# culiver/VAR

Hardware: AMD Instinct MI355X
Metric: 256x256 images/sec (CFG=1.5) VAR-d16 (higher is better)
Workload: dtype f32

## Files before the change

include/var_hip.h:

```cpp
#ifndef VAR_HIP_H
#define VAR_HIP_H

#include <stdint.h>

#ifdef __cplusplus
extern "C" {
#endif

#define VARHIP_EINVAL (-1)

typedef void* varhip_stream_t;

const char* varhip_version(void);

#define VARHIP_EPI_NONE 0
#define VARHIP_EPI_GELU 1
#define VARHIP_EPI_RESID 2
int varhip_gemm_nt_f32(const float* A, int64_t lda, const float* W, int64_t ldw, const float* bias,
                       float* out, int64_t ldo, int M, int N, int K, int epi,
                       const float* resid, int64_t ldr, const float* gamma, int64_t ldg, int rows_per_group,
                       int bias_per_row, int batch, int64_t sA, int64_t sW, int64_t sO, varhip_stream_t stream);

int varhip_silu_f32(const float* x, float* y, int64_t n, varhip_stream_t stream);

// ... 49 lines not shown
int varhip_upconv_pack_f32(const float* w, float* w_phase, int Cin, int Cout, varhip_stream_t stream);
int varhip_upconv_phase_f32(const float* in, const float* w_phase, const float* bias, float* out,
                            int B, int H, int W, int Cin, int Cout, varhip_stream_t stream);
int varhip_upconv_phase_gn_f32(const float* in, const float* w_phase, const float* bias, float* out, double* gn_part,
                               int B, int H, int W, int Cin, int Cout, varhip_stream_t stream);

int64_t varhip_gn_scratch_elems(int B, int HW, int C, int G);
int varhip_gn_stats_f32(const float* x, float* stats, double* scratch, int B, int HW, int C, int G, float eps, varhip_stream_t stream);
int varhip_gn_apply_f32(const float* x, const float* stats, const float* gamma, const float* beta, float* out,
                        int B, int HW, int C, int G, int silu, varhip_stream_t stream);

int varhip_gn_silu_conv_out_f32(const float* x, const float* stats, const float* gamma, const float* beta, const float* w, const float* bias,
                                float* out, int B, int H, int W, int Cin, int Cout, int G, int out_mode, varhip_stream_t stream);

int varhip_softmax_rows_f32(const float* x, float* out, int64_t rows, int n, float scale, varhip_stream_t stream);

int varhip_nchw_to_nhwc_f32(const float* in, float* out, int B, int C, int HW, varhip_stream_t stream);
int varhip_nhwc_to_nchw_f32(const float* in, float* out, int B, int C, int HW, varhip_stream_t stream);

int varhip_conv_gn_blocks(int H, int W, int Cout, int phase);
int varhip_conv3x3_gn_nhwc_f32(const float* in, const float* w, const float* bias, const float* resid, float* out, double* gn_part,
                               int B, int H, int W, int Cin, int Cout, int up2, varhip_stream_t stream);
int varhip_gn_stats_part_f32(const double* gn_part, float* stats, int B, int nblk, int HW, int C, int G, float eps, varhip_stream_t stream);
int varhip_conv3x3_s2_nhwc_f32(const float* in, const float* w, const float* bias, float* out,
                               int B, int H, int W, int Cin, int Cout, varhip_stream_t stream);
int varhip_nchw_to_nhwc_pad_f32(const float* in, float* out, int B, int C, int HW, int Cpad, varhip_stream_t stream);
int varhip_area_pool_f32(const float* f, float* pooled, int B, int P, int pq, int Cv, varhip_stream_t stream);
int varhip_word_embed_f32(const float* pooled, const float* word_w, const float* word_b, const float* lvl_pos,
                          float* x_out, int B, int lq, int C, int Cv, varhip_stream_t stream);
int varhip_quant_residual_f32(const int64_t* idx, const float* codebook, const int32_t* tap_idx, const float* tap_w,
                              const float* phi_w, const float* phi_b, float ratio, float* up, float* f_hat, float* f_rest,
                              int B, int pn, int P, int Cv, varhip_stream_t stream);

int varhip_token_select_i64(const uint8_t* keep, const int64_t* gt, const int64_t* sampled, int64_t* out, int64_t n, varhip_stream_t stream);

int varhip_neighbor_table_f32(const float* codebook, int V, int D, int n, int32_t* nbr_idx, float* nbr_dist, varhip_stream_t stream);
int varhip_smooth_select_f32(const float* logits, const int64_t* gt, const int32_t* nbr_idx, const float* nbr_dist, int n,
                             int cand_count, int use_thr, float thr, float ratio, int B, int l, int V, double t_cfg,
                             int64_t* idx_out, float* maxval_out, float* distlp_out, float* cfg_out, varhip_stream_t stream);

int varhip_token_loglik_f32(const float* logits, const int64_t* gt, int64_t ld_gt, int images, int classes, int l, int V,
                            int with_uncond, float ca, float cb, float* out, int64_t ld_out_img, int64_t ld_out_cls, varhip_stream_t stream);

int varhip_code_dist_f32(const float* codebook, int V, int D, float* out, varhip_stream_t stream);
int varhip_token_score_f32(const float* logits, const int64_t* gt, int64_t ld_gt, int images, int classes, int l, int V,
                           int with_uncond, float ca, float cb, int mode, int param, float thr, const float* dist, int64_t ld_dist,
// ... 56 lines not shown
                              void* out, int M, int C, int rows_per_group, float eps, varhip_stream_t stream);
int varhip_adaln_block_bf16(float* x, float* x2, void* xn16, void* q16, void* att16, void* hid16, const float* ada, int64_t ld_ada,
                           const void* qkv_w16, const float* qkv_b, const float* scale_mul, float plain_scale, int l2norm,
                           const void* proj_w16, const float* proj_b, const void* fc1_w16, const float* fc1_b,
                           const void* fc2_w16, const float* fc2_b, void* kcache16, void* vcache16,
                           int B2, int l, int C, int H, int hidden, int pos0, int Lmax, float eps, varhip_stream_t stream);
int varhip_conv3x3_nhwc_bf16(const void* in, const void* w, const float* bias, const void* resid, void* out, double* gn_part,
                            int B, int H, int W, int Cin, int Cout, int out_mode, varhip_stream_t stream);
int varhip_upconv_phase_bf16(const void* in, const void* w_phase, const float* bias, void* out, double* gn_part,
                            int B, int H, int W, int Cin, int Cout, varhip_stream_t stream);
int varhip_gnconv3x3_nhwc_bf16(const void* in, const float* table, int silu,
                               const void* w, const float* bias, const void* resid, void* out, double* gn_part,
                               int B, int H, int W, int Cin, int Cout, varhip_stream_t stream);
int varhip_conv16_force_tile(int wm);
int varhip_gn_stats_bf16(const void* x, float* stats, double* scratch, int B, int HW, int C, int G, float eps, varhip_stream_t stream);
int varhip_gn_apply_bf16(const void* x, const float* stats, const float* gamma, const float* beta, void* out,
                        int B, int HW, int C, int G, int silu, varhip_stream_t stream);
int varhip_gn_silu_conv_out_bf16(const void* x, const float* stats, const float* gamma, const float* beta, const void* w, const float* bias,
                                 float* out, int B, int H, int W, int Cin, int Cout, int G, int out_mode, varhip_stream_t stream);
int varhip_cast_f32_to_bf16(const float* in, void* out, int64_t n, varhip_stream_t stream);
int varhip_cast_bf16_to_f32(const void* in, float* out, int64_t n, varhip_stream_t stream);


#define VARHIP_NFAM 15
int varhip_timing_enable(int on);
int varhip_timing_select(int family_mask);
int varhip_timing_reset(void);
int varhip_timing_read(double* ms, double* flops, double* bytes, int64_t* launches);
const char* varhip_timing_name(int family);

#ifdef __cplusplus
}
#endif
#endif
```

var_amd/abi.py:

```python
import ctypes as C

P = C.c_void_p
I = C.c_int
L = C.c_int64
F = C.c_float
D = C.c_double

SIGNATURES = {
    'gemm_nt_f32':       [P, L, P, L, P, P, L, I, I, I, I, P, L, P, L, I, I, I, L, L, L],
    'silu_f32':          [P, P, L],
    'add_bcast_f32':     [P, P, P, I, I],
    'ln_modulate_f32':   [P, P, L, P, L, P, I, I, I, F],
    'qkv_prep_f32':      [P, P, F, I, P, P, P, I, I, I, I, I],
    'attn_cached_f32':   [P, P, P, P, I, I, I, I, I],
    'cfg_sample_f32':    [P, P, P, P, I, I, I, D, I, D],
    'quant_accum_f32':   [P, P, P, P, P, P, F, P, P, I, I, I, I],
    'next_map_f32':      [P, P, P, P, P, P, I, I, I, I, I],
    'lvl_pos_f32':       [P, P, P, P, I, I],
    'first_map_f32':     [P, P, I, P, P, P, P, I, I, I],
    'conv3x3_nhwc_f32':  [P, P, P, P, P, I, I, I, I, I, I, I],
    'gn_stats_f32':      [P, P, P, I, I, I, I, F],
    'gn_apply_f32':      [P, P, P, P, P, I, I, I, I, I],
    'softmax_rows_f32':  [P, P, L, I, F],
    'nchw_to_nhwc_f32':  [P, P, I, I, I],
# ... 21 lines not shown

SIGNATURES_F16 = {
    'gemm_nt_f16':       [P, L, P, L, P, P, L, I, I, I, I, I, P, L, I, P, L, I, I, L, L, L],
    'gemm_qkv_f16':      [P, L, P, L, P, I, I, I, P, F, I, P, P, P, I, I, I, I, I],
    'attn_cached_f16':   [P, P, P, P, I, I, I, I, I],
    'ln_modulate_f16out': [P, P, L, P, L, P, I, I, I, F],
    'adaln_block_f16':   [P, P, P, P, P, P, P, L, P, P, P, F, I, P, P, P, P, P, P, P, P, I, I, I, I, I, I, I, F],
    'conv3x3_nhwc_f16':  [P, P, P, P, P, P, I, I, I, I, I, I],
    'upconv_phase_f16':  [P, P, P, P, P, I, I, I, I, I],
    'gnconv3x3_nhwc_f16': [P, P, I, P, P, P, P, P, I, I, I, I, I],
    'gn_stats_f16':      [P, P, P, I, I, I, I, F],
    'gn_apply_f16':      [P, P, P, P, P, I, I, I, I, I],
    'gn_silu_conv_out_f16': [P, P, P, P, P, P, P, I, I, I, I, I, I, I],
    'cast_f32_to_f16':   [P, P, L],
    'cast_f16_to_f32':   [P, P, L],
}

SIGNATURES_HIP_ONLY = {
    'gn_scale_shift_f32': [P, P, P, P, I, I, I],
    'gn_silu_conv_out_f32': [P, P, P, P, P, P, P, I, I, I, I, I, I, I],
    'token_loglik_f32':  [P, P, L, I, I, I, I, I, F, F, P, L, L],
    'code_dist_f32':     [P, I, I, P],
    'token_score_f32':   [P, P, L, I, I, I, I, I, F, F, I, I, F, P, L, P, L, L],
}

SIGNATURES_BF16 = {k.replace('_f16out', '_bf16out').replace('_to_f16', '_to_bf16').replace('cast_f16_', 'cast_bf16_').replace('_f16', '_bf16'): v
                   for k, v in SIGNATURES_F16.items()}

EPI_NONE, EPI_GELU, EPI_RESID = 0, 1, 2
EINVAL = -1


def bind(lib, prefix: str, with_stream: bool):
    fns = {}
    table = dict(SIGNATURES)
    if with_stream:
        table.update(SIGNATURES_F16)
        table.update(SIGNATURES_BF16)
        table.update(SIGNATURES_HIP_ONLY)
    for name, args in table.items():
        fn = getattr(lib, prefix + name)
        fn.argtypes = list(args) + ([P] if with_stream else [])
        fn.restype = I
        fns[name] = fn
    gs = getattr(lib, prefix + 'gn_scratch_elems')
    gs.argtypes = [I, I, I, I]
# ... 17 lines not shown
```

var_amd/csrc/common.h:

```cpp
#pragma once
#include <hip/hip_runtime.h>
#include <stdint.h>
#include <stdlib.h>
#include "../../include/var_hip.h"
#include "../../include/var_math.h"

typedef float f32x2 __attribute__((ext_vector_type(2)));
__device__ __forceinline__ f32x2 vh_exp_pair(f32x2 x) {
    const f32x2 xc = {__builtin_fminf(x[0], 88.0f), __builtin_fminf(x[1], 88.0f)};
    const f32x2 t = xc * 1.44269504088896341f;
    const f32x2 n = {__builtin_rintf(t[0]), __builtin_rintf(t[1])};
    f32x2 r = __builtin_elementwise_fma(n, (f32x2)(-0.693145751953125f), xc);
    r = __builtin_elementwise_fma(n, (f32x2)(-1.42860682030941723212e-6f), r);
    f32x2 q = (f32x2)(1.9875691500e-4f);
    q = __builtin_elementwise_fma(q, r, (f32x2)(1.3981999507e-3f));
    q = __builtin_elementwise_fma(q, r, (f32x2)(8.3334519073e-3f));
    q = __builtin_elementwise_fma(q, r, (f32x2)(4.1665795894e-2f));
    q = __builtin_elementwise_fma(q, r, (f32x2)(1.6666665459e-1f));
    q = __builtin_elementwise_fma(q, r, (f32x2)(5.0000001201e-1f));
    const f32x2 y = __builtin_elementwise_fma(q, r * r, r) + 1.0f;
    f32x2 o;
    o[0] = (x[0] > -87.0f) ? __builtin_ldexpf(y[0], (int)n[0]) : 0.0f;
    o[1] = (x[1] > -87.0f) ? __builtin_ldexpf(y[1], (int)n[1]) : 0.0f;
    return o;
// ... 4 lines not shown
    const f32x2 u = (x + x3 * 0.044715f) * 0.7978845608028654f;
    const f32x2 d = vh_exp_pair(u * -2.0f) + 1.0f;
    return f32x2{x[0] / d[0], x[1] / d[1]};
}

typedef float f32x4 __attribute__((ext_vector_type(4)));
typedef float f32x16 __attribute__((ext_vector_type(16)));

#define VH_FAM_GEMM 0
#define VH_FAM_CONV 1
#define VH_FAM_ATTN 2
#define VH_FAM_SAMPLER 3
#define VH_FAM_LN 4
#define VH_FAM_QKV 5
#define VH_FAM_GN 6
#define VH_FAM_OTHER 7
#define VH_FAM_GEMM_SMALL 8
#define VH_FAM_CONV_SMALL 9
#define VH_FAM_GEMM16 10
#define VH_FAM_GEMM16_SMALL 11
#define VH_FAM_CONV16H 12
#define VH_FAM_CONV16_SMALL 13
#define VH_FAM_ATTN16 14

int vh_timing_on(int fam);
void vh_timing_begin(int fam, hipStream_t s, double flops, double bytes);
void vh_timing_end(int fam, hipStream_t s);

struct VhScope {
    int fam; hipStream_t s; bool on;
    VhScope(int f, hipStream_t st, double flops, double bytes) : fam(f), s(st), on(vh_timing_on(f) != 0) { if (on) vh_timing_begin(fam, s, flops, bytes); }
    ~VhScope() { if (on) vh_timing_end(fam, s); }
};

static inline int vh_launch_status() {
    hipError_t e = hipGetLastError();
    return e == hipSuccess ? 0 : -(1000 + (int)e);
}

template <int CTRL> __device__ __forceinline__ float vh_mov_dpp(float v) {
    return __int_as_float(__builtin_amdgcn_mov_dpp(__float_as_int(v), CTRL, 0xF, 0xF, true));
}
__device__ __forceinline__ float vh_lane_xor4(float v) {
    const float up = vh_mov_dpp<0x104>(v), dn = vh_mov_dpp<0x114>(v);
    return (threadIdx.x & 4) ? dn : up;
}
__device__ __forceinline__ float vh_wave_sum(float p) {
    { const auto r = __builtin_amdgcn_permlane32_swap(__float_as_uint(p), __float_as_uint(p), false, false); p = __uint_as_float(r[0]) + __uint_as_float(r[1]); }
    { const auto r = __builtin_amdgcn_permlane16_swap(__float_as_uint(p), __float_as_uint(p), false, false); p = __uint_as_float(r[0]) + __uint_as_float(r[1]); }
    p = p + vh_mov_dpp<0x128>(p);
    p = p + vh_lane_xor4(p);
    p = p + vh_mov_dpp<0x4E>(p);
    p = p + vh_mov_dpp<0xB1>(p);
    return p;
}
__device__ __forceinline__ float vh_wave_max(float p) {
// ... 23 lines not shown
```

var_amd/csrc/gemm.hip:

```cpp
#include "common.h"

struct GemmP {
    const float* A; const float* W; const float* bias; float* out; const float* resid; const float* gamma;
    int64_t lda, ldw, ldo, ldr, ldg, sA, sW, sO;
    int M, N, K, epi, rows_per_group, bias_per_row;
    int H, Wd, Cin, up2, out_mode, Hi, Wi;
    int tilesM, tilesN;
    int evec;
    const float* q_smul; float* q_out; float* q_kc; float* q_vc; float q_plain; int q_l2, q_l, q_pos0, q_Lmax;
    double* gn_part;
};

__global__ void __launch_bounds__(256) k_gemm_any(GemmP p) {
    const int lane = threadIdx.x & 63, wave = threadIdx.x >> 6, r = lane & 31, h = lane >> 5;
    const int tm = blockIdx.x / p.tilesN, tn = blockIdx.x - tm * p.tilesN, bz = blockIdx.z;
    const int m0 = tm * 64 + (wave >> 1) * 32, n0 = tn * 64 + (wave & 1) * 32;
    const int ma = m0 + r, nb = n0 + r;
    const float* a = p.A + (int64_t)bz * p.sA + (int64_t)(ma < p.M ? ma : 0) * p.lda;
    const float* w = p.W + (int64_t)bz * p.sW + (int64_t)(nb < p.N ? nb : 0) * p.ldw;
    float* Ob = p.out + (int64_t)bz * p.sO;
    f32x16 acc;
#pragma unroll
    for (int e = 0; e < 16; ++e) acc[e] = 0.f;
    for (int k0 = 0; k0 < p.K; k0 += 2) {
// ... 10 lines not shown
        float v = acc[e];
        if (p.bias) v = v + (p.bias_per_row ? p.bias[m] : p.bias[n]);
        if (p.epi == VARHIP_EPI_GELU) v = vm_gelu_tanh(v);
        else if (p.epi == VARHIP_EPI_RESID) {
            if (p.gamma) v = v * p.gamma[(int64_t)(m / p.rows_per_group) * p.ldg + n];
            v = p.resid[(int64_t)m * p.ldr + n] + v;
        }
        Ob[(int64_t)m * p.ldo + n] = v;
    }
}

__device__ __attribute__((aligned(128))) float g_zero_row[32];

template <int N> __device__ __forceinline__ void vh_waitcnt_barrier() { asm volatile("s_waitcnt vmcnt(%0)\n\ts_barrier" ::"n"(N) : "memory"); }
template <int MAXA, int PER> __device__ __forceinline__ void vh_wait_dma_and_barrier(int ahead) {
    if constexpr (MAXA == 0) vh_waitcnt_barrier<0>();
    else { if (ahead >= MAXA) vh_waitcnt_barrier<MAXA * PER>(); else vh_wait_dma_and_barrier<MAXA - 1, PER>(ahead); }
}

__device__ __forceinline__ void vh_dma16(const void* base, uint32_t voff, uint32_t lds) {
    asm volatile("s_mov_b32 m0, %2\n\ts_nop 0\n\tglobal_load_lds_dwordx4 %0, %1" : : "v"(voff), "s"(base), "s"(lds) : "memory", "m0");
}

__device__ __forceinline__ void vh_dma16_buf(__amdgpu_buffer_rsrc_t rsrc, uint32_t voff, uint32_t soff, uint32_t lds) {
    asm volatile("s_mov_b32 m0, %3\n\ts_nop 0\n\tbuffer_load_dwordx4 %0, %1, %2 offen lds"
                 : : "v"(voff), "s"(rsrc), "s"(__builtin_amdgcn_readfirstlane(soff)), "s"(__builtin_amdgcn_readfirstlane(lds)) : "memory", "m0");
}

__device__ __forceinline__ void vh_dma16_ptr(const void* src, uint32_t lds) {
    asm volatile("s_mov_b32 m0, %1\n\ts_nop 0\n\tglobal_load_lds_dwordx4 %0, off" : : "v"(src), "s"(lds) : "memory", "m0");
}

template <int TMW, int TNW, bool CONV, int NST = 2, bool GATHER = false>
__global__ void __launch_bounds__(256) k_dma_gemm(GemmP p) {
    constexpr int BK = 32, BM = TMW * 32, BN = TNW * 32, STAGE = (BM + BN) * BK;
    constexpr int NIA = BM / 32, NIB = BN / 32;
    extern __shared__ __attribute__((aligned(16))) float smem[];
    const int tid = threadIdx.x, lane = tid & 63, wave = __builtin_amdgcn_readfirstlane(tid >> 6);
    const int wm = wave >> 1, wn = wave & 1;
    int tm_, tn_;
    {
        const int nwg = p.tilesM * p.tilesN, bid = blockIdx.x;
        const int q = nwg >> 3, rem = nwg & 7, xcd = bid & 7, loc = bid >> 3;
        const int lin = (xcd < rem ? xcd * (q + 1) : rem * (q + 1) + (xcd - rem) * q) + loc;
        const int GM = 8, width = GM * p.tilesN, group = lin / width, first = group * GM;
        const int gsz = (p.tilesM - first) < GM ? (p.tilesM - first) : GM;
        tm_ = first + (lin % width) % gsz;
        tn_ = (lin % width) / gsz;
    }
    const int m0 = tm_ * BM, n0 = tn_ * BN;
// ... 601 lines not shown
```

var_amd/csrc/timing.hip:

```cpp
#include "common.h"
#include <mutex>
#include <vector>

namespace {
struct Rec { hipEvent_t a, b; int fam; };
std::mutex g_mu;
int g_on = 0;
int g_mask = ~0;
std::vector<Rec> g_pool;
size_t g_used = 0;
double g_ms[VARHIP_NFAM], g_flops[VARHIP_NFAM], g_bytes[VARHIP_NFAM];
int64_t g_n[VARHIP_NFAM];
const size_t kMaxRecs = 1 << 15;

void drain_locked() {
    for (size_t i = 0; i < g_used; ++i) {
        float ms = 0.f;
        if (hipEventSynchronize(g_pool[i].b) == hipSuccess && hipEventElapsedTime(&ms, g_pool[i].a, g_pool[i].b) == hipSuccess)
            g_ms[g_pool[i].fam] += ms;
    }
    g_used = 0;
}
}

// ... 35 lines not shown
int varhip_timing_select(int family_mask) { std::lock_guard<std::mutex> lk(g_mu); g_mask = family_mask; return 0; }

int varhip_timing_reset(void) {
    std::lock_guard<std::mutex> lk(g_mu);
    drain_locked();
    for (int i = 0; i < VARHIP_NFAM; ++i) { g_ms[i] = g_flops[i] = g_bytes[i] = 0.0; g_n[i] = 0; }
    return 0;
}

int varhip_timing_read(double* ms, double* flops, double* bytes, int64_t* launches) {
    std::lock_guard<std::mutex> lk(g_mu);
    drain_locked();
    for (int i = 0; i < VARHIP_NFAM; ++i) {
        if (ms) ms[i] = g_ms[i];
        if (flops) flops[i] = g_flops[i];
        if (bytes) bytes[i] = g_bytes[i];
        if (launches) launches[i] = g_n[i];
    }
    return VARHIP_NFAM;
}

const char* varhip_timing_name(int f) {
    static const char* names[VARHIP_NFAM] = {"gemm", "conv3x3", "attn", "sampler", "ln", "qkv_prep", "gn", "other", "gemm_small", "conv_small",
                                               "gemm16", "gemm16_small", "conv16h", "conv16_small", "attn16"};
    return (f >= 0 && f < VARHIP_NFAM) ? names[f] : "?";
}

}
```

var_amd/engine.py:

```python
from __future__ import annotations

import math
import os
from typing import Dict, List, Optional

import numpy as np
import torch

from . import hip
from .abi import EPI_GELU, EPI_NONE, EPI_RESID


def bicubic_taps(pn: int, P: int):
    f = np.float32
    A = f(-0.75)
    scale = f(pn) / f(P)
    src = scale * (np.arange(P, dtype=np.float32) + f(0.5)) - f(0.5)
    i0 = np.floor(src)
    t = (src - i0).astype(np.float32)

    def near(x):
        return ((A + f(2)) * x - (A + f(3))) * x * x + f(1)

    def far(x):
# ... 69 lines not shown
    def invalidate(self):
        self._sig = None

    def _pack(self):
        w = {}
        for k, v in self.vae.state_dict().items():
            if not k.startswith(self.PREFIXES) or not torch.is_floating_point(v):
                continue
            v = _chk(v.detach(), k)
            if v.dim() == 4 and v.shape[-1] == 3:
                v = v.permute(0, 2, 3, 1).contiguous()
                if v.shape[3] % 32:
                    pad = torch.zeros(v.shape[0], 3, 3, (v.shape[3] + 31) // 32 * 32, dtype=v.dtype, device=v.device)
                    pad[..., :v.shape[3]] = v
                    v = pad
                w[k] = v
            elif v.dim() == 4:
                w[k] = v.reshape(v.shape[0], v.shape[1])
            else:
                w[k] = v
        return w


class DecoderEngine(_VaeOps):

    PREFIXES = ('decoder.', 'post_quant_conv.')
    precision = 'f32'
    unfused_tail = False

    def set_precision(self, precision: str):
        if precision not in PRECISIONS:
            raise ValueError(f"precision must be one of {PRECISIONS}")
        self.precision = precision

    def refresh(self):
        sig = self._signature()
        if sig == self._sig:
            return
        self._retire()
        w = self._pack()
        for k in [k for k in w if k.endswith('.upsample.conv.weight')]:
            cout, _, _, cin = w[k].shape
            wp = torch.empty(4, cout, 2, 2, cin, dtype=torch.float32, device=w[k].device)
            hip.call('upconv_pack_f32', w[k], wp, cin, cout)
            w[k[:-len('weight')] + 'phase'] = wp
        self.w = w
        self.w16s = {}
        self.nlev = 1 + max(int(k.split('.')[2]) for k in w if k.startswith('decoder.up.'))
        self._sig = sig
        self._built()

    def _ensure16(self, prec):
        if prec not in self.w16s:
            self._wait_ready()
            self.w16s[prec] = {k: v.to(DT16[prec]).contiguous() for k, v in self.w.items()
                               if (k.endswith('.weight') or k.endswith('.phase')) and v.dim() >= 2 and '.norm' not in k}
            self._built()
        self.w16, self.sfx, self.dt16 = self.w16s[prec], prec, DT16[prec]

    def _part_buffer(self, B, nblk, Cout, dev):
        return torch.empty((B, nblk, Cout, 2), dtype=torch.float64, device=dev)

    def conv3(self, x, key, B, Hh, Ww, up2=0, resid=None, out_mode=0, stats=False):
        wt = self.w[key + '.weight']
        Cout, Cin = wt.shape[0], wt.shape[3]
        out = torch.empty((B, Cout, Hh, Ww) if out_mode else (B, Hh, Ww, Cout), dtype=torch.float32, device=x.device)
        nblk = hip.conv_gn_blocks(Hh, Ww, Cout) if (stats and out_mode == 0) else 0
        if nblk:
            part = self._part_buffer(B, nblk, Cout, x.device)
            hip.call('conv3x3_gn_nhwc_f32', x, wt, self.w[key + '.bias'], resid, out, part, B, Hh, Ww, Cin, Cout, up2)
            self._gn_part = (out, part, nblk)
        else:
            hip.call('conv3x3_nhwc_f32', x, wt, self.w[key + '.bias'], resid, out, B, Hh, Ww, Cin, Cout, up2, out_mode)
        return out

    def gn_stats(self, x, B, HW):
        return self._stats_from(x, B, HW, 'gn_stats_f32')

    def gn(self, x, key, B, HW, silu):
        stats = self.gn_stats(x, B, HW)
        out = torch.empty_like(x)
        hip.call('gn_apply_f32', x, stats, self.w[key + '.weight'], self.w[key + '.bias'], out, B, HW, x.shape[-1], 32, int(silu))
        return out

    def tail(self, h, B, Hh, Ww, denorm):
        wt = self.w['decoder.conv_out.weight']
        Cout, Cin = wt.shape[0], wt.shape[3]
        if Hh % 8 == 0 and Ww % 32 == 0 and Cin % 32 == 0 and Cout <= 4 and (10 * 34 * 36 + 4 * Cin) * 4 <= 64 * 1024 and not self.unfused_tail:
            stats = self.gn_stats(h, B, Hh * Ww)
            out = torch.empty((B, Cout, Hh, Ww), dtype=torch.float32, device=h.device)
            hip.call('gn_silu_conv_out_f32', h, stats, self.w['decoder.norm_out.weight'], self.w['decoder.norm_out.bias'], wt,
                     self.w['decoder.conv_out.bias'], out, B, Hh, Ww, Cin, Cout, 32, 1 if denorm else 2)
            return out
        h = self.gn(h, 'decoder.norm_out', B, Hh * Ww, True)
        return self.conv3(h, 'decoder.conv_out', B, Hh, Ww, out_mode=1 if denorm else 2)

    def lin(self, x2d, key, resid=None):
# ... 28 lines not shown
        p = torch.empty_like(s)
        hip.call('softmax_rows_f32', s, p, B * HW, HW, float(np.float32(int(Cc) ** (-0.5))))
        o = torch.empty((B * HW, Cc), dtype=torch.float32, device=dev)
        hip.call('gemm_nt_f32', p, HW, vt, HW, None, o, Cc, HW, Cc, HW, EPI_NONE, None, 0, None, 0, 1, 0, B, HW * HW, Cc * HW, HW * Cc)
        return self.lin(o, pre + '.proj_out', resid=x.view(B * HW, Cc)).view(B, Hh, Ww, Cc)

    def flops_per_image_reference(self, P: int) -> float:
        self.refresh()
        w = self.w
        def c3(key, hw): co, _, _, ci = w[key + '.weight'].shape; return 2.0 * hw * co * 9 * ci
        def c1(key, hw): co, ci = w[key + '.weight'].shape; return 2.0 * hw * co * ci
        def res(pre, hw): return c3(pre + '.conv1', hw) + c3(pre + '.conv2', hw) + (c1(pre + '.nin_shortcut', hw) if (pre + '.nin_shortcut.weight') in w else 0.0)
        def att(pre, hw): c = w[pre + '.proj_out.weight'].shape[0]; return c1(pre + '.qkv', hw) + c1(pre + '.proj_out', hw) + 2.0 * 2 * hw * hw * c
        hw = P * P
        f = c3('post_quant_conv', hw) + c3('decoder.conv_in', hw) + res('decoder.mid.block_1', hw) + att('decoder.mid.attn_1', hw) + res('decoder.mid.block_2', hw)
        for lev in reversed(range(self.nlev)):
            for ib in range(3):
                f += res(f'decoder.up.{lev}.block.{ib}', hw)
                if f'decoder.up.{lev}.attn.{ib}.norm.weight' in w: f += att(f'decoder.up.{lev}.attn.{ib}', hw)
            if lev != 0:
                hw *= 4; f += c3(f'decoder.up.{lev}.upsample.conv', hw)
        return f + c3('decoder.conv_out', hw)

    def flops_per_image_executed(self, P: int) -> float:
        f = self.flops_per_image_reference(P)
        hw = P * P
        for lev in reversed(range(self.nlev)):
            if lev != 0:
                hw *= 4
                co, _, _, ci = self.w[f'decoder.up.{lev}.upsample.conv.weight'].shape
                f -= 2.0 * hw * co * 5 * ci
        return f

    def conv3_16(self, x, key, B, Hh, Ww, resid=None, out_mode=0, stats=False):
        wt = self.w16[key + '.weight']
        Cout, Cin = wt.shape[0], wt.shape[3]
        out = torch.empty((B, Cout, Hh, Ww), dtype=torch.float32, device=x.device) if out_mode else torch.empty((B, Hh, Ww, Cout), dtype=self.dt16, device=x.device)
        nblk = hip.conv_gn_blocks(Hh, Ww, Cout) if (stats and out_mode == 0 and Cout % 4 == 0) else 0
        part = self._part_buffer(B, nblk, Cout, x.device) if nblk else None
        hip.call('conv3x3_nhwc_' + self.sfx, x, wt, self.w[key + '.bias'], resid, out, part, B, Hh, Ww, Cin, Cout, out_mode)
        if nblk: self._gn_part = (out, part, nblk)
        return out

    def gn_stats16(self, x, B, HW):
        return self._stats_from(x, B, HW, 'gn_stats_' + self.sfx)

    def gn16(self, x, key, B, HW, silu):
        stats = self.gn_stats16(x, B, HW)
        out = torch.empty_like(x)
        hip.call('gn_apply_' + self.sfx, x, stats, self.w[key + '.weight'], self.w[key + '.bias'], out, B, HW, x.shape[-1], 32, int(silu))
        return out

# ... 79 lines not shown
        h = self.resblock16(h, 'decoder.mid.block_1', B, Hh, Ww)
        h = self.attnblock16(h, 'decoder.mid.attn_1', B, Hh, Ww)
        h = self.resblock16(h, 'decoder.mid.block_2', B, Hh, Ww)
        for lev in reversed(range(self.nlev)):
            for ib in range(3):
                h = self.resblock16(h, f'decoder.up.{lev}.block.{ib}', B, Hh, Ww)
                if f'decoder.up.{lev}.attn.{ib}.norm.weight' in self.w:
                    h = self.attnblock16(h, f'decoder.up.{lev}.attn.{ib}', B, Hh, Ww)
            if lev != 0:
                Hh, Ww = 2 * Hh, 2 * Ww
                key = f'decoder.up.{lev}.upsample.conv'
                wp = self.w16[key + '.phase']
                up = torch.empty((B, Hh, Ww, wp.shape[1]), dtype=self.dt16, device=h.device)
                nblk = hip.conv_gn_blocks(Hh, Ww, wp.shape[1], phase=True)
                part = self._part_buffer(B, nblk, wp.shape[1], h.device) if nblk else None
                hip.call('upconv_phase_' + self.sfx, h, wp, self.w[key + '.bias'], up, part, B, Hh, Ww, wp.shape[4], wp.shape[1])
                self._gn_part = (up, part, nblk) if nblk else None
                h = up
        return self.tail16(h, B, Hh, Ww, denorm)

    def decode_nhwc(self, f_hat: torch.Tensor, denorm: bool = True, precision: Optional[str] = None) -> torch.Tensor:
        self.refresh()
        prec = precision or self.precision
        if prec != 'f32':
            self._ensure16(prec)
            self._wait_ready()
            return self._decode16(f_hat, denorm)
        self._wait_ready()
        B, P = f_hat.shape[0], f_hat.shape[1]
        Hh = Ww = P
        h = self.conv3(f_hat, 'post_quant_conv', B, Hh, Ww)
        h = self.conv3(h, 'decoder.conv_in', B, Hh, Ww, stats=True)
        h = self.resblock(h, 'decoder.mid.block_1', B, Hh, Ww)
        h = self.attnblock(h, 'decoder.mid.attn_1', B, Hh, Ww)
        h = self.resblock(h, 'decoder.mid.block_2', B, Hh, Ww)
        for lev in reversed(range(self.nlev)):
            for ib in range(3):
                h = self.resblock(h, f'decoder.up.{lev}.block.{ib}', B, Hh, Ww)
                if f'decoder.up.{lev}.attn.{ib}.norm.weight' in self.w:
                    h = self.attnblock(h, f'decoder.up.{lev}.attn.{ib}', B, Hh, Ww)
            if lev != 0:
                Hh, Ww = 2 * Hh, 2 * Ww
                key = f'decoder.up.{lev}.upsample.conv'
                wp = self.w[key + '.phase']
                up = torch.empty((B, Hh, Ww, wp.shape[1]), dtype=torch.float32, device=h.device)
                nblk = hip.conv_gn_blocks(Hh, Ww, wp.shape[1], phase=True)
# ... 235 lines not shown
    _wait_ready = _VaeOps._wait_ready

    def _ensure16(self):
        prec = self.precision
        if prec == 'f32' or prec in self.w['b16']:
            return
        self._wait_ready()
        dt = DT16[prec]
        self.w['b16'][prec] = [{k + '16': d[k].to(dt).contiguous() for k in ('qkv_w', 'proj_w', 'fc1_w', 'fc2_w')} for d in self.w['blocks']]
        self.w['head_w16'][prec] = self.w['head_w'].to(dt).contiguous()
        self._built()

    def resolve_precision(self) -> str:
        if self.policy == 'auto':
            self.precision = AUTOCAST_PRECISION.get(torch.get_autocast_dtype('cuda'), 'f32') if torch.is_autocast_enabled('cuda') else 'f32'
        else:
            self.precision = self.policy
        return self.precision

    def set_precision(self, precision: str):
        if precision not in PRECISIONS + ('auto',):
            raise ValueError(f"precision must be one of {PRECISIONS + ('auto',)}")
        self.policy = precision
        if precision != 'auto' and precision != self.precision:
            self.precision = precision
            self._ws = {k: v for k, v in self._ws.items() if k[2] == precision}
            self._ws_tf = {k: v for k, v in self._ws_tf.items() if k[2] == precision}

    def invalidate(self):
        self._sig = None
        self.dec.invalidate()

    def workspace(self, B: int):
        sid = int(torch.cuda.current_stream().cuda_stream)
        ws = self._ws.get((B, sid, self.precision))
        dev = self.var.pos_start.device
        if ws is not None and ws['dev'] == dev:
            return ws
        var = self.var
        C, L, H, V, Cv, P = var.C, var.L, var.num_heads, var.V, var.Cvae, var.patch_nums[-1]
        lmax = max(p * p for p in var.patch_nums)
        M = 2 * B * lmax
        hid = var.blocks[0].ffn.fc1.weight.shape[0]
        e = lambda *s, dt=torch.float32: torch.empty(*s, dtype=dt, device=dev)
        act = DT16.get(self.precision, torch.float32)
        ws = dict(dev=dev, x=e(M, C), x2=e(M, C), xn=e(M, C, dt=act), q=e(M, C, dt=act), att=e(M, C, dt=act), hid=e(M, hid, dt=act), logits=e(M, V),
# ... 375 lines not shown
```

var_amd/hip.py:

```python
import ctypes
import os

from . import abi

_HERE = os.path.dirname(os.path.abspath(__file__))
LIB_PATH = os.environ.get('VARHIP_LIB') or os.path.join(_HERE, 'libvar_hip.so')


class VarHipError(RuntimeError):
    pass


class _Lib:
    def __init__(self):
        if not os.path.exists(LIB_PATH):
            raise VarHipError(f'{LIB_PATH} not found: build it with `python -c "import __graft_entry__ as g; g.build()"` '
                              f'(or `make -C var_amd/csrc`). There is no CPU/PyTorch fallback for the sampling path.')
        self.so = ctypes.CDLL(LIB_PATH)
        self.fn = abi.bind(self.so, 'varhip_', with_stream=True)
        so = self.so
        so.varhip_timing_enable.argtypes = [ctypes.c_int]; so.varhip_timing_enable.restype = ctypes.c_int
        so.varhip_timing_reset.argtypes = []; so.varhip_timing_reset.restype = ctypes.c_int
        so.varhip_timing_read.argtypes = [ctypes.c_void_p] * 4; so.varhip_timing_read.restype = ctypes.c_int
        so.varhip_timing_name.argtypes = [ctypes.c_int]; so.varhip_timing_name.restype = ctypes.c_char_p
# ... 29 lines not shown
    return ctypes.c_void_p(torch.cuda.current_stream().cuda_stream)


def call(name: str, *args, stream=None):
    L = lib()
    st = current_stream() if stream is None else stream
    rc = L.fn[name](*[_arg(a) for a in args], st)
    if rc != 0:
        raise VarHipError(f'varhip_{name} returned {rc}' + (' (VARHIP_EINVAL: unsupported shape/argument)' if rc == abi.EINVAL else ' (HIP launch error %d)' % (-rc - 1000)))


def gn_scratch_elems(B, HW, C, G) -> int:
    return int(lib().fn['gn_scratch_elems'](B, HW, C, G))


def conv_gn_blocks(H, W, Cout, phase=False) -> int:
    return int(lib().fn['conv_gn_blocks'](H, W, Cout, 1 if phase else 0))


def conv16_gn_fusable(B, H, W, Cin, Cout) -> bool:
    return bool(lib().fn['conv16_gn_fusable'](B, H, W, Cin, Cout))


NFAM = 15


def timing_enable(on: bool, families=None):
    so = lib().so
    mask = -1
    if families is not None:
        names = [so.varhip_timing_name(i).decode() for i in range(NFAM)]
        mask = sum(1 << names.index(f) for f in families)
    so.varhip_timing_select(mask)
    so.varhip_timing_enable(1 if on else 0)


def timing_reset():
    lib().so.varhip_timing_reset()


def timing_read():
    n = abi_nfam = NFAM
    ms = (ctypes.c_double * n)(); fl = (ctypes.c_double * n)(); by = (ctypes.c_double * n)(); ln = (ctypes.c_int64 * n)()
    lib().so.varhip_timing_read(ms, fl, by, ln)
    return {lib().so.varhip_timing_name(i).decode(): dict(ms=ms[i], flops=fl[i], bytes=by[i], launches=int(ln[i])) for i in range(abi_nfam)}
```

Before: 136.3.

## Add Winograd F(2x2,3x3) f32 conv kernel for decoder resnet convs

Adds a Winograd F(2x2,3x3) NHWC f32 conv kernel that uses fp32 MFMA, LDS DMA staging with double buffering, and a fused bias, residual and GroupNorm partial-stats epilogue. Filters are pre-transformed on the host when weights load. The decoder resnet conv1/conv2 layers use it by default whenever the shape fits (HW≥256, multiples of 16 and 32). The goal is to cut the multiply count of the f32 decoder convs, at the cost of extra transform arithmetic and small numerical differences. FLOP accounting is also adjusted.

After: 154.0 (median of 6 runs). 1.13x the previous value.

```diff
diff --git a/include/var_hip.h b/include/var_hip.h
--- a/include/var_hip.h
+++ b/include/var_hip.h
@@ -95,6 +95,8 @@
 int varhip_conv3x3_gn_nhwc_f32(const float* in, const float* w, const float* bias, const float* resid, float* out, double* gn_part,
                                int B, int H, int W, int Cin, int Cout, int up2, varhip_stream_t stream);
 int varhip_gn_stats_part_f32(const double* gn_part, float* stats, int B, int nblk, int HW, int C, int G, float eps, varhip_stream_t stream);
+int varhip_conv3x3_wino_nhwc_f32(const float* in, const float* u, const float* bias, const float* resid, float* out, double* gn_part,
+                                 int B, int H, int W, int Cin, int Cout, varhip_stream_t stream);
 int varhip_conv3x3_s2_nhwc_f32(const float* in, const float* w, const float* bias, float* out,
                                int B, int H, int W, int Cin, int Cout, varhip_stream_t stream);
 int varhip_nchw_to_nhwc_pad_f32(const float* in, float* out, int B, int C, int HW, int Cpad, varhip_stream_t stream);
@@ -197,7 +199,7 @@
 int varhip_cast_bf16_to_f32(const void* in, float* out, int64_t n, varhip_stream_t stream);
 
 
-#define VARHIP_NFAM 15
+#define VARHIP_NFAM 16
 int varhip_timing_enable(int on);
 int varhip_timing_select(int family_mask);
 int varhip_timing_reset(void);
diff --git a/var_amd/abi.py b/var_amd/abi.py
--- a/var_amd/abi.py
+++ b/var_amd/abi.py
@@ -67,6 +67,7 @@
     'token_loglik_f32':  [P, P, L, I, I, I, I, I, F, F, P, L, L],
     'code_dist_f32':     [P, I, I, P],
     'token_score_f32':   [P, P, L, I, I, I, I, I, F, F, I, I, F, P, L, P, L, L],
+    'conv3x3_wino_nhwc_f32': [P, P, P, P, P, P, I, I, I, I, I],
 }
 
 SIGNATURES_BF16 = {k.replace('_f16out', '_bf16out').replace('_to_f16', '_to_bf16').replace('cast_f16_', 'cast_bf16_').replace('_f16', '_bf16'): v
diff --git a/var_amd/csrc/common.h b/var_amd/csrc/common.h
--- a/var_amd/csrc/common.h
+++ b/var_amd/csrc/common.h
@@ -50,6 +50,7 @@
 #define VH_FAM_CONV16H 12
 #define VH_FAM_CONV16_SMALL 13
 #define VH_FAM_ATTN16 14
+#define VH_FAM_CONV_WINO 15
 
 int vh_timing_on(int fam);
 void vh_timing_begin(int fam, hipStream_t s, double flops, double bytes);
@@ -60,6 +61,11 @@
     VhScope(int f, hipStream_t st, double flops, double bytes) : fam(f), s(st), on(vh_timing_on(f) != 0) { if (on) vh_timing_begin(fam, s, flops, bytes); }
     ~VhScope() { if (on) vh_timing_end(fam, s); }
 };
+
+__device__ __forceinline__ void vh_dma16_buf(__amdgpu_buffer_rsrc_t rsrc, uint32_t voff, uint32_t soff, uint32_t lds) {
+    asm volatile("s_mov_b32 m0, %3\n\ts_nop 0\n\tbuffer_load_dwordx4 %0, %1, %2 offen lds"
+                 : : "v"(voff), "s"(rsrc), "s"(__builtin_amdgcn_readfirstlane(soff)), "s"(__builtin_amdgcn_readfirstlane(lds)) : "memory", "m0");
+}
 
 static inline int vh_launch_status() {
     hipError_t e = hipGetLastError();
diff --git a/var_amd/csrc/gemm.hip b/var_amd/csrc/gemm.hip
--- a/var_amd/csrc/gemm.hip
+++ b/var_amd/csrc/gemm.hip
@@ -56,10 +56,6 @@
     asm volatile("s_mov_b32 m0, %2\n\ts_nop 0\n\tglobal_load_lds_dwordx4 %0, %1" : : "v"(voff), "s"(base), "s"(lds) : "memory", "m0");
 }
 
-__device__ __forceinline__ void vh_dma16_buf(__amdgpu_buffer_rsrc_t rsrc, uint32_t voff, uint32_t soff, uint32_t lds) {
-    asm volatile("s_mov_b32 m0, %3\n\ts_nop 0\n\tbuffer_load_dwordx4 %0, %1, %2 offen lds"
-                 : : "v"(voff), "s"(rsrc), "s"(__builtin_amdgcn_readfirstlane(soff)), "s"(__builtin_amdgcn_readfirstlane(lds)) : "memory", "m0");
-}
 
 __device__ __forceinline__ void vh_dma16_ptr(const void* src, uint32_t lds) {
     asm volatile("s_mov_b32 m0, %1\n\ts_nop 0\n\tglobal_load_lds_dwordx4 %0, off" : : "v"(src), "s"(lds) : "memory", "m0");
diff --git a/var_amd/csrc/timing.hip b/var_amd/csrc/timing.hip
--- a/var_amd/csrc/timing.hip
+++ b/var_amd/csrc/timing.hip
@@ -81,7 +81,8 @@
 
 const char* varhip_timing_name(int f) {
     static const char* names[VARHIP_NFAM] = {"gemm", "conv3x3", "attn", "sampler", "ln", "qkv_prep", "gn", "other", "gemm_small", "conv_small",
-                                               "gemm16", "gemm16_small", "conv16h", "conv16_small", "attn16"};
+                                               "gemm16", "gemm16_small", "conv16h", "conv16_small", "attn16",
+                                               "conv_wino"};
     return (f >= 0 && f < VARHIP_NFAM) ? names[f] : "?";
 }
 
diff --git a/var_amd/csrc/winograd.hip b/var_amd/csrc/winograd.hip
--- /dev/null
+++ b/var_amd/csrc/winograd.hip
@@ -0,0 +1,191 @@
+#include "common.h"
+
+namespace {
+
+constexpr int WG_PT = 18;
+constexpr int WG_NDMA = 21;
+constexpr int WG_STAGE = WG_NDMA * 16 * 64;
+constexpr int WG_ZSTR = 20;
+constexpr int WG_LDS = 2 * WG_STAGE;
+static_assert(8 * 64 * WG_ZSTR * 4 <= WG_LDS, "epilogue exchange must fit in the K-loop stages");
+
+struct WinoP {
+    const float* in; const float* u; const float* bias; const float* resid; float* out; double* gn_part;
+    int H, W, Cin, Cout, ncg, pw, ppi;
+};
+
+__device__ __forceinline__ void wg_wait_dma_barrier() { asm volatile("s_waitcnt vmcnt(0)\n\ts_barrier" ::: "memory"); }
+
+__device__ __forceinline__ int wg_swz(int pix) { return (pix >> 1) & 3; }
+
+__global__ void __launch_bounds__(256, 2) k_conv3x3_wino(WinoP p) {
+    extern __shared__ __attribute__((aligned(16))) float smem[];
+    const int tid = threadIdx.x, lane = tid & 63, wave = __builtin_amdgcn_readfirstlane(tid >> 6);
+    const int r16 = lane & 15, kq = lane >> 4;
+    int lin;
+    {
+        const int nwg = gridDim.x, bid = blockIdx.x, q = nwg >> 3, rem = nwg & 7, xcd = bid & 7, loc = bid >> 3;
+        lin = (xcd < rem ? xcd * (q + 1) : rem * (q + 1) + (xcd - rem) * q) + loc;
+    }
+    const int cg = lin % p.ncg, pidx = lin / p.ncg, b = pidx / p.ppi, pi = pidx - b * p.ppi, py = pi / p.pw, px = pi - py * p.pw;
+    const int y0 = py * 16, x0 = px * 16, c0 = cg * 32;
+    const int H = p.H, W = p.W, Cin = p.Cin, Cout = p.Cout, nk = Cin >> 4;
+
+    const int64_t img = (int64_t)H * W * Cin;
+    const __amdgpu_buffer_rsrc_t rsrc = __builtin_amdgcn_make_buffer_rsrc((void*)(p.in + (int64_t)b * img), 0, (int)(img * 4), 0x00020000);
+    uint32_t doff[6];
+#pragma unroll
+    for (int i = 0; i < 6; ++i) {
+        const int pix = (wave + 4 * i) * 16 + (lane >> 2), c = lane & 3;
+        const int yy = y0 - 1 + pix / WG_PT, xx = x0 - 1 + pix % WG_PT;
+        const bool ok = pix < WG_PT * WG_PT && (unsigned)yy < (unsigned)H && (unsigned)xx < (unsigned)W;
+        doff[i] = ok ? (uint32_t)((((int64_t)yy * W + xx) * Cin + ((c ^ wg_swz(pix)) << 2)) * 4) : 0x80000000u;
+    }
+    const uint32_t lds0 = (uint32_t)(uintptr_t)(__attribute__((address_space(3))) void*)smem;
+    auto dma = [&](int kt, int st) {
+#pragma unroll
+        for (int i = 0; i < 6; ++i)
+            if (wave + 4 * i < WG_NDMA) vh_dma16_buf(rsrc, doff[i], (uint32_t)kt * 64u, lds0 + st * WG_STAGE + (wave + 4 * i) * 1024);
+    };
+
+    const uint32_t ustr_xi = (uint32_t)nk * Cout * 64, ustr_kt = (uint32_t)Cout * 64;
+    const __amdgpu_buffer_rsrc_t ursrc = __builtin_amdgcn_make_buffer_rsrc((void*)p.u, 0, (int)(16 * ustr_xi), 0x00020000);
+    const uint32_t uoff = (uint32_t)((c0 + r16) * 16 + 4 * kq) * 4u;
+    auto load_u = [&](int kt, f32x4 (&u)[4][2]) {
+#pragma unroll
+        for (int j = 0; j < 4; ++j)
+#pragma unroll
+            for (int cb = 0; cb < 2; ++cb)
+                u[j][cb] = __builtin_bit_cast(f32x4, __builtin_amdgcn_raw_buffer_load_b128(
+                    ursrc, uoff, __builtin_amdgcn_readfirstlane((uint32_t)(4 * wave + j) * ustr_xi + (uint32_t)kt * ustr_kt + cb * 1024u), 0));
+    };
+
+    const int ra = wave == 3 ? 1 : (wave == 2 ? 2 : wave), rb = wave == 0 ? 2 : (wave == 1 ? 2 : (wave == 2 ? 1 : 3));
+    const float sg = wave == 1 ? 1.0f : -1.0f;
+    uint32_t roff[2][4];
+#pragma unroll
+    for (int c = 0; c < 4; ++c) {
+        const int pa = (2 * (r16 >> 3) + ra) * WG_PT + 2 * (r16 & 7) + c, pb = (2 * (r16 >> 3) + rb) * WG_PT + 2 * (r16 & 7) + c;
+        roff[0][c] = (uint32_t)(pa * 64 + ((kq ^ wg_swz(pa)) << 4));
+        roff[1][c] = (uint32_t)(pb * 64 + ((kq ^ wg_swz(pb)) << 4));
+    }
+
+    f32x4 acc[4][4][2];
+#pragma unroll
+    for (int j = 0; j < 4; ++j)
+#pragma unroll
+        for (int tb = 0; tb < 4; ++tb)
+#pragma unroll
+            for (int cb = 0; cb < 2; ++cb) acc[j][tb][cb] = f32x4{0.f, 0.f, 0.f, 0.f};
+
+    auto compute = [&](int st, const f32x4 (&u)[4][2]) {
+        const char* sb = (const char*)smem + st * WG_STAGE;
+#pragma unroll
+        for (int tb = 0; tb < 4; ++tb) {
+            f32x4 da[4], db[4];
+#pragma unroll
+            for (int c = 0; c < 4; ++c) {
+                da[c] = *(const f32x4*)(sb + roff[0][c] + tb * 72 * 64);
+                db[c] = *(const f32x4*)(sb + roff[1][c] + tb * 72 * 64);
+            }
+#pragma unroll
+            for (int s = 0; s < 4; ++s) {
+                float e[4];
+#pragma unroll
+                for (int c = 0; c < 4; ++c) e[c] = __builtin_fmaf(sg, db[c][s], da[c][s]);
+                const float v[4] = {e[0] - e[2], e[1] + e[2], e[2] - e[1], e[1] - e[3]};
+#pragma unroll
+                for (int j = 0; j < 4; ++j)
+#pragma unroll
+                    for (int cb = 0; cb < 2; ++cb) acc[j][tb][cb] = __builtin_amdgcn_mfma_f32_16x16x4f32(u[j][cb][s], v[j], acc[j][tb][cb], 0, 0, 0);
+            }
+            __builtin_amdgcn_sched_barrier(0);
+        }
+    };
+
+    f32x4 u[4][2];
+    dma(0, 0);
+    wg_wait_dma_barrier();
+    int kt = 0;
+    for (; kt + 1 < nk; kt += 2) {
+        load_u(kt, u); dma(kt + 1, 1);
+        compute(0, u);
+        wg_wait_dma_barrier();
+        load_u(kt + 1, u); if (kt + 2 < nk) dma(kt + 2, 0);
+        compute(1, u);
+        wg_wait_dma_barrier();
+    }
+    if (kt < nk) { load_u(kt, u); compute(0, u); wg_wait_dma_barrier(); }
+
+    float* zb = smem;
+    const int et = tid & 63, eq = tid >> 6;
+    const int ety = et >> 3, etx = et & 7;
+    const int64_t obase = (((int64_t)b * H + y0 + 2 * ety) * W + x0 + 2 * etx) * Cout;
+    const int nblk = p.gn_part ? (H * W) >> 7 : 0;
+#pragma unroll
+    for (int cb = 0; cb < 2; ++cb) {
+#pragma unroll
+        for (int tb = 0; tb < 4; ++tb) {
+            const f32x4 m0 = acc[0][tb][cb], m1 = acc[1][tb][cb], m2 = acc[2][tb][cb], m3 = acc[3][tb][cb];
+            const f32x4 z0 = (m0 + m1) + m2, z1 = (m1 - m2) - m3;
+            const int t = tb * 16 + r16;
+            *(f32x4*)(zb + ((wave * 2 + 0) * 64 + t) * WG_ZSTR + 4 * kq) = z0;
+            *(f32x4*)(zb + ((wave * 2 + 1) * 64 + t) * WG_ZSTR + 4 * kq) = z1;
+        }
+        __syncthreads();
+        f32x4 z[4][2];
+#pragma unroll
+        for (int i = 0; i < 4; ++i)
+#pragma unroll
+            for (int bb = 0; bb < 2; ++bb) z[i][bb] = *(const f32x4*)(zb + ((i * 2 + bb) * 64 + et) * WG_ZSTR + 4 * eq);
+        const int co = c0 + cb * 16 + 4 * eq;
+        const f32x4 b4 = *(const f32x4*)(p.bias + co);
+        double gs[4] = {0.0, 0.0, 0.0, 0.0}, gq[4] = {0.0, 0.0, 0.0, 0.0};
+#pragma unroll
+        for (int a = 0; a < 2; ++a)
+#pragma unroll
+            for (int bb = 0; bb < 2; ++bb) {
+                const f32x4 yv = a == 0 ? (z[0][bb] + z[1][bb]) + z[2][bb] : (z[1][bb] - z[2][bb]) - z[3][bb];
+                f32x4 v = yv + b4;
+                const int64_t o = obase + ((int64_t)a * W + bb) * Cout + co;
+                if (p.resid) v = *(const f32x4*)(p.resid + o) + v;
+                *(f32x4*)(p.out + o) = v;
+#pragma unroll
+                for (int e = 0; e < 4; ++e) { const double d = (double)v[e]; gs[e] += d; gq[e] += d * d; }
+            }
+        if (p.gn_part) {
+#pragma unroll
+            for (int off = 16; off >= 1; off >>= 1)
+#pragma unroll
+                for (int e = 0; e < 4; ++e) { gs[e] += __shfl_xor(gs[e], off, 64); gq[e] += __shfl_xor(gq[e], off, 64); }
+            if ((lane & 31) == 0) {
+                double* g = p.gn_part + (((int64_t)b * nblk + 2 * pi + (lane >> 5)) * Cout + co) * 2;
+#pragma unroll
+                for (int e = 0; e < 4; ++e) { g[2 * e] = gs[e]; g[2 * e + 1] = gq[e]; }
+            }
+        }
+        if (cb == 0) __syncthreads();
+    }
+}
+
+}
+
+extern "C" int varhip_conv3x3_wino_nhwc_f32(const float* in, const float* u, const float* bias, const float* resid, float* out, double* gn_part,
+                                            int B, int H, int W, int Cin, int Cout, varhip_stream_t stream) {
+    if (!in || !u || !bias || !out || B <= 0 || H <= 0 || W <= 0 || Cin <= 0 || Cout <= 0) return VARHIP_EINVAL;
+    if ((H & 15) || (W & 15) || (Cin & 31) || (Cout & 31)) return VARHIP_EINVAL;
+    if ((((uintptr_t)in | (uintptr_t)u | (uintptr_t)bias | (uintptr_t)out | (uintptr_t)resid) & 15)) return VARHIP_EINVAL;
+    if ((int64_t)H * W * Cin * 4 >= (1ll << 31) || 64ll * Cin * Cout >= (1ll << 31) || (int64_t)B * H * W >= (1ll << 31))
+        return VARHIP_EINVAL;
+    const int ppi = (H / 16) * (W / 16), ncg = Cout / 32;
+    const int64_t nwg = (int64_t)B * ppi * ncg;
+    if (nwg >= (1ll << 31)) return VARHIP_EINVAL;
+    WinoP p{};
+    p.in = in; p.u = u; p.bias = bias; p.resid = resid; p.out = out; p.gn_part = gn_part;
+    p.H = H; p.W = W; p.Cin = Cin; p.Cout = Cout; p.ncg = ncg; p.pw = W / 16; p.ppi = ppi;
+    const double npix = (double)B * H * W;
+    VhScope scope(VH_FAM_CONV_WINO, (hipStream_t)stream, 2.0 * (npix / 4.0) * 16.0 * Cin * Cout,
+                  4.0 * (npix * Cin + npix * Cout * (resid ? 2.0 : 1.0) + 16.0 * Cin * Cout));
+    hipLaunchKernelGGL(k_conv3x3_wino, dim3((unsigned)nwg), dim3(256), WG_LDS, (hipStream_t)stream, p);
+    return vh_launch_status();
+}
diff --git a/var_amd/engine.py b/var_amd/engine.py
--- a/var_amd/engine.py
+++ b/var_amd/engine.py
@@ -115,11 +115,24 @@
         return w
 
 
+_WINO_G = ((1.0, 0.0, 0.0), (0.5, 0.5, 0.5), (0.5, -0.5, 0.5), (0.0, 0.0, 1.0))
+
+
+def wino_filter(w: torch.Tensor) -> torch.Tensor:
+    co, _, _, ci = w.shape
+    G = torch.tensor(_WINO_G, dtype=torch.float64, device=w.device)
+    u = torch.einsum('ik,jl,oklc->ijoc', G, G, w.double()).float()
+    return u.reshape(16, co, ci // 16, 16).permute(0, 2, 1, 3).contiguous()
+
+
 class DecoderEngine(_VaeOps):
 
     PREFIXES = ('decoder.', 'post_quant_conv.')
     precision = 'f32'
     unfused_tail = False
+    winograd = os.environ.get('VARHIP_WINOGRAD', '1') != '0'
+    WINO_MIN_HW = 16 * 16
+    flops_precision = None
 
     def set_precision(self, precision: str):
         if precision not in PRECISIONS:
@@ -137,6 +150,8 @@
             wp = torch.empty(4, cout, 2, 2, cin, dtype=torch.float32, device=w[k].device)
             hip.call('upconv_pack_f32', w[k], wp, cin, cout)
             w[k[:-len('weight')] + 'phase'] = wp
+        for k in [k for k in w if k.endswith(('.conv1.weight', '.conv2.weight'))]:
+            w[k[:-len('weight')] + 'wino'] = wino_filter(w[k])
         self.w = w
         self.w16s = {}
         self.nlev = 1 + max(int(k.split('.')[2]) for k in w if k.startswith('decoder.up.'))
@@ -159,13 +174,20 @@
         Cout, Cin = wt.shape[0], wt.shape[3]
         out = torch.empty((B, Cout, Hh, Ww) if out_mode else (B, Hh, Ww, Cout), dtype=torch.float32, device=x.device)
         nblk = hip.conv_gn_blocks(Hh, Ww, Cout) if (stats and out_mode == 0) else 0
-        if nblk:
+        if up2 == 0 and out_mode == 0 and self.winograd and (key + '.wino') in self.w and self.wino_ok(Hh, Ww, Cin, Cout):
+            part = self._part_buffer(B, nblk, Cout, x.device) if nblk else None
+            hip.call('conv3x3_wino_nhwc_f32', x, self.w[key + '.wino'], self.w[key + '.bias'], resid, out, part, B, Hh, Ww, Cin, Cout)
+            if nblk: self._gn_part = (out, part, nblk)
+        elif nblk:
             part = self._part_buffer(B, nblk, Cout, x.device)
             hip.call('conv3x3_gn_nhwc_f32', x, wt, self.w[key + '.bias'], resid, out, part, B, Hh, Ww, Cin, Cout, up2)
             self._gn_part = (out, part, nblk)
         else:
             hip.call('conv3x3_nhwc_f32', x, wt, self.w[key + '.bias'], resid, out, B, Hh, Ww, Cin, Cout, up2, out_mode)
         return out
+
+    def wino_ok(self, Hh, Ww, Cin, Cout):
+        return Hh * Ww >= self.WINO_MIN_HW and Hh % 16 == 0 and Ww % 16 == 0 and Cin % 32 == 0 and Cout % 32 == 0
 
     def gn_stats(self, x, B, HW):
         return self._stats_from(x, B, HW, 'gn_stats_f32')
@@ -240,12 +262,22 @@
                 hw *= 4; f += c3(f'decoder.up.{lev}.upsample.conv', hw)
         return f + c3('decoder.conv_out', hw)
 
-    def flops_per_image_executed(self, P: int) -> float:
+    def flops_per_image_executed(self, P: int, precision: Optional[str] = None) -> float:
+        prec = precision or self.flops_precision or self.precision
         f = self.flops_per_image_reference(P)
-        hw = P * P
+        hw, side = P * P, P
+        def wino(pre, hw, side):
+            d = 0.0
+            for c in ('.conv1', '.conv2'):
+                co, _, _, ci = self.w[pre + c + '.weight'].shape
+                if prec == 'f32' and self.winograd and self.wino_ok(side, side, ci, co): d += 2.0 * hw * co * 5 * ci
+            return d
+        f -= wino('decoder.mid.block_1', hw, side) + wino('decoder.mid.block_2', hw, side)
         for lev in reversed(range(self.nlev)):
+            for ib in range(3):
+                f -= wino(f'decoder.up.{lev}.block.{ib}', hw, side)
             if lev != 0:
-                hw *= 4
+                hw *= 4; side *= 2
                 co, _, _, ci = self.w[f'decoder.up.{lev}.upsample.conv.weight'].shape
                 f -= 2.0 * hw * co * 5 * ci
         return f
@@ -371,6 +403,7 @@
     def decode_nhwc(self, f_hat: torch.Tensor, denorm: bool = True, precision: Optional[str] = None) -> torch.Tensor:
         self.refresh()
         prec = precision or self.precision
+        self.flops_precision = prec
         if prec != 'f32':
             self._ensure16(prec)
             self._wait_ready()
@@ -652,6 +685,8 @@
         if precision not in PRECISIONS + ('auto',):
             raise ValueError(f"precision must be one of {PRECISIONS + ('auto',)}")
         self.policy = precision
+        if precision != 'auto':
+            self.dec.flops_precision = precision
         if precision != 'auto' and precision != self.precision:
             self.precision = precision
             self._ws = {k: v for k, v in self._ws.items() if k[2] == precision}
diff --git a/var_amd/hip.py b/var_amd/hip.py
--- a/var_amd/hip.py
+++ b/var_amd/hip.py
@@ -75,7 +75,7 @@
     return bool(lib().fn['conv16_gn_fusable'](B, H, W, Cin, Cout))
 
 
-NFAM = 15
+NFAM = 16
 
 
 def timing_enable(on: bool, families=None):
```
